# winlaic/ZipVoice

Hardware: AMD Instinct MI355X
Metric: generated mel-frames/s (whole job) + RTF, ZipVoice 123M N_steps=16 batch=32/GPU (higher is better)
Workload: dtype bf16; 1 GPU; C2: ZipVoice 123M, N_steps=16, batch=32/GPU x (3 s prompt + 10 s generated; T=1219 frames), CFG g=1.0 (64 decoder rows per GPU), t_shift=0.5; model=zipvoice (zipvoice_base.json, synthetic seeded weights), global_batch=32, seq_len=1219, parallelism=dp1

## Files before the change

### include/zipvoice_hip.h

```cpp
#ifndef ZIPVOICE_HIP_H
#define ZIPVOICE_HIP_H

#include <stdint.h>

#ifdef __cplusplus
extern "C" {
#endif

typedef struct zv_engine* zv_handle;

enum zv_variant { ZV_ZIPVOICE = 0, ZV_DISTILL = 1, ZV_DIALOG = 2, ZV_DIALOG_STEREO = 3 };
enum zv_precision { ZV_FP32 = 0, ZV_BF16 = 1, ZV_MIXED = 2, ZV_FP8 = 3 };

#define ZV_MAX_STACKS 8

typedef struct {
  int variant;
  int precision;
  int feat_dim;
  int num_stacks;
  int downsampling_factor[ZV_MAX_STACKS];
  int num_layers[ZV_MAX_STACKS];
  int cnn_module_kernel[ZV_MAX_STACKS];
  int fm_decoder_dim, fm_decoder_feedforward_dim, fm_decoder_num_heads;
// ... 94 lines not shown
enum zv_stackedge_kind { ZV_SE_DOWNSAMPLE = 0, ZV_SE_UPSAMPLE = 1, ZV_SE_MASK = 2, ZV_SE_ENTRY = 3, ZV_SE_BIASNORM = 4 };
typedef struct {
  int kind, B, L, C, ds, guard, rows_per_group;
  float log_scale;
  const float* x; const float* w; const float* nb; const float* orig; const float* rowvec;
  const uint8_t* mask;
  float* out;
  uint8_t* mout;
  uint16_t* h; uint16_t* l; uint16_t* h2; uint16_t* l2; int64_t ldact;
  uint8_t* q2; uint8_t* qs2; int64_t ldq;
  int launch[8];
  int num_cus;
} zv_stackedge_check_args;
int zv_stackedge_check(zv_stackedge_check_args* a);

enum zv_bigvgan_check_kind { ZV_BV_FILTER = 0, ZV_BV_ACT = 1, ZV_BV_CONV = 2, ZV_BV_CONVT = 3, ZV_BV_AVG = 4,
                             ZV_BV_POST = 5, ZV_BV_IM2COL = 6, ZV_BV_STEP = 7 };
typedef struct {
  int kind, split, mode, guard;
  int B, Lmax, Ls, halo, scale;
  int C, Cout, ks, d, u, n, layout, flag;
  float div, sub, bias0;
  unsigned stale;
  const int* lens;
  const float* x; const float* x1; const float* x2;
  const float* w; const float* bias; const float* alpha; const float* ibeta;
  const float* w2; const float* bias2; const float* alpha2; const float* ibeta2;
  const float* taps; const float* resid;
  const uint16_t* ah; const uint16_t* al;
  float* out; uint16_t* oh; uint16_t* ol; int64_t ld;
// ... 125 lines not shown
```

### zipvoice_amd/csrc/zv_checks.inc

```
#pragma once

namespace {

struct ChkDev {
  std::vector<void*> ptrs;
  void* raw(size_t bytes) {
    void* p = nullptr;
    ZV_CHECK(ZV_BLOCKING(hipMalloc(&p, bytes + 256)));
    ptrs.push_back(p);
    return p;
  }
  template <typename T> T* make(size_t n) { return reinterpret_cast<T*>(raw(n * sizeof(T))); }
  template <typename T> T* zero(size_t n) {
    T* d = make<T>(n);
    ZV_CHECK(ZV_BLOCKING(hipMemset(d, 0, n * sizeof(T))));
    return d;
  }
  template <typename T> T* up(const T* host, size_t n) {
    T* d = make<T>(n);
    ZV_CHECK(ZV_BLOCKING(hipMemcpy(d, host, n * sizeof(T), hipMemcpyHostToDevice)));
    return d;
  }
  template <typename T> void down(T* host, const T* dev, size_t n) {
    ZV_CHECK(ZV_BLOCKING(hipMemcpy(host, dev, n * sizeof(T), hipMemcpyDeviceToHost)));
// ... 696 lines not shown
    }
    ZV_LAUNCH_CHECK();
    ZV_CHECK(ZV_BLOCKING(hipDeviceSynchronize()));
    dev.down(a->out, o, (size_t)(M + 2 * G) * C);
    down16(a->h, h, M); down16(a->l, l, M); down16(a->h2, h2, M); down16(a->l2, l2, M);
    if (q2) {
      dev.down(a->q2, q2, (size_t)(M + 2 * G) * a->ldq);
      dev.down(a->qs2, qs2, (size_t)(M + 2 * G) * ldqs);
    }
  }
  memcpy(a->launch, rec, sizeof(rec));
  a->num_cus = zv_num_cus();
  ZV_API_END
}

}

namespace {
inline unsigned chk_hash(size_t i, unsigned seed) {
  unsigned x = (unsigned)i * 2654435761u ^ (seed * 0x9E3779B9u + 0x7F4A7C15u);
  x ^= x >> 13; x *= 0x5bd1e995u; x ^= x >> 15;
  return x;
}
inline uint16_t chk_stale16(size_t i, unsigned seed) {
  const unsigned x = chk_hash(i, seed);
  return (uint16_t)(0x3C00u | (x & 0x3FFu) | ((x >> 16 & 1u) << 15));
}
inline float chk_stale32(size_t i, unsigned seed) {
  const unsigned x = chk_hash(i, seed);
  return ((x >> 20 & 1u) ? -1.f : 1.f) * (1.f + (float)(x & 0xFFFFu) / 16384.f);
// ... 258 lines not shown
```

### zipvoice_amd/csrc/zv_elem.inc

```
#pragma once
#include "zv_common.h"
#include "zv_gemm.inc"

__global__ void zv_build_input_kernel(const float* x, const float* tc, const float* sc,
                                      bf16* oh, bf16* ol, long ld, int B, int T, int Fx, int Ft,
                                      int Fs, int ncopies, int zero_speech_uncond) {
  const int Fin = Fx + Ft + Fs;
  const long total = (long)ncopies * B * T * Fin;
  for (long idx = blockIdx.x * (long)blockDim.x + threadIdx.x; idx < total;
       idx += (long)gridDim.x * blockDim.x) {
    const int f = (int)(idx % Fin);
    const long row = idx / Fin;
    const long bt = row % ((long)B * T);
    const int copy = (int)(row / ((long)B * T));
    const bool uncond = (ncopies == 2 && copy == 0);
    float v;
    if (f < Fx) v = x[bt * Fx + f];
    else if (f < Fx + Ft) v = uncond ? 0.f : tc[bt * Ft + (f - Fx)];
    else v = (uncond && zero_speech_uncond) ? 0.f : sc[bt * Fs + (f - Fx - Ft)];
    split_store(oh, ol, row * ld + f, v);
  }
}

__global__ __launch_bounds__(256) void zv_build_input4_kernel(
// ... 659 lines not shown

__global__ void zv_mask_downsample_kernel(const uint8_t* in, uint8_t* out, int B, int L,
                                          int dL, int ds) {
  const int idx = blockIdx.x * blockDim.x + threadIdx.x;
  if (idx >= B * dL) return;
  const int b = idx / dL, i = idx % dL;
  out[idx] = in[(long)b * L + (long)i * ds];
}

__global__ void zv_copy_u8_kernel(const uint8_t* in, uint8_t* out, long n, int copies) {
  const long idx = blockIdx.x * (long)blockDim.x + threadIdx.x;
  if (idx >= n * copies) return;
  out[idx] = in[idx % n];
}

__global__ void zv_embed_kernel(const int64_t* tok, const float* table, bf16* oh, bf16* ol,
                                long ld, long n, int C) {
  const long total = n * C;
  for (long idx = blockIdx.x * (long)blockDim.x + threadIdx.x; idx < total;
       idx += (long)gridDim.x * blockDim.x) {
    const long r = idx / C;
    const int c = (int)(idx % C);
    split_store(oh, ol, r * ld + c, table[tok[r] * C + c]);
  }
}

__global__ void zv_spk_add_kernel(float* emb, const int8_t* spk, const float* table, long n,
                                  int C) {
  const long total = n * C;
  for (long idx = blockIdx.x * (long)blockDim.x + threadIdx.x; idx < total;
// ... 36 lines not shown
```

### zipvoice_amd/csrc/zv_engine.hip

```cpp
#include <math.h>
#include <stdlib.h>
#include <string.h>

#include <map>
#include <memory>
#include <mutex>
#include <string>
#include <exception>
#include <functional>
#include <tuple>
#include <vector>


#include "zv_common.h"
#include "zv_gemm.inc"
#include "zv_gemm256.inc"
#include "zv_ffn.inc"
#include "zv_attn.inc"
#include "zv_elem.inc"
#include "zv_flash.inc"
#include "zv_flash2.inc"
#include "zv_weights.inc"
#include "zv_linear.inc"
#include "../../include/zipvoice_hip.h"
// ... 67 lines not shown
    a.ld = ld;
    a.h = with16 ? h.get<bf16>((size_t)rows * ld) : nullptr;
    a.l = split ? l.get<bf16>((size_t)rows * ld) : nullptr;
    if (fp8) {
      a.ldq = round_up(cols ? cols : ld, MX8_KSTEP);
      a.q = q.get<uint8_t>((size_t)rows * a.ldq);
      a.qs = qs.get<uint8_t>((size_t)rows * a.ldq / MX8_BLOCK);
    }
    return a;
  }
  size_t bytes() const { return h.bytes + l.bytes + q.bytes + qs.bytes; }
};

struct Workspace {
  DBuf main, dsrc, cur, temb0, temb1, tstack, tvec, gvec, posP, mask2, maskds, vout, stats;
  ActBuf xin, main_a, dsrc_a, cur_a, qkp, W, hidden, na_y, na_xt, na_o, sa_vt, sa_o, glu, dw, emb;
  ActBuf cur8;
  ActBuf dwo;
  DBuf ffn_part, ffn_flag;
  static constexpr int POSP_STACKS = 8;
  DBuf posPs[POSP_STACKS];
  struct PosPKey { int L = -1, nl = 0; const void* w = nullptr; const void* buf = nullptr; };
  PosPKey posk[POSP_STACKS];
  size_t bytes() const {
    size_t s = 0;
    for (const DBuf& b : posPs) s += b.bytes;
    for (const DBuf* b : {&main, &dsrc, &cur, &temb0, &temb1, &tstack, &tvec, &gvec, &posP, &mask2,
                          &maskds, &vout, &stats, &ffn_part, &ffn_flag})
      s += b->bytes;
    for (const ActBuf* b : {&xin, &main_a, &dsrc_a, &cur_a, &qkp, &W, &hidden, &na_y, &na_xt, &na_o,
                            &sa_vt, &sa_o, &glu, &dw, &emb, &cur8, &dwo})
      s += b->bytes();
    return s;
  }
};

constexpr int ZV_STREAM_SET = 4;
struct StreamSet { hipStream_t s[ZV_STREAM_SET] = {}; int dev = -1; };
static std::mutex g_stream_pool_mu;
static std::vector<StreamSet>& stream_pool_free() { static std::vector<StreamSet> v; return v; }
static StreamSet acquire_stream_set() {
  int dev = 0;
  ZV_CHECK(hipGetDevice(&dev));
  {
    std::lock_guard<std::mutex> lock(g_stream_pool_mu);
    auto& fr = stream_pool_free();
    for (size_t i = 0; i < fr.size(); ++i)
      if (fr[i].dev == dev) {
// ... 48 lines not shown
    auto envi = [](const char* k, int d) { const char* v = getenv(k); return v ? atoi(v) : d; };
    materialize_attn = envi("ZV_ATTN_MATERIALIZE", 0) == 1;
    graph_mode = envi("ZV_GRAPH", 2);
    sa_tp = envi("ZV_SA_TP", 1);
    fp8_fuse = envi("ZV_FP8_FUSE", 7);
    ffn_fused = envi("ZV_FFN", 2);
    ffn_min_rows = envi("ZV_FFN_MIN_ROWS", 15000);
    ffn_persist = envi("ZV_FFN_PERSIST", 1);
    split_streams = envi("ZV_SPLIT_STREAMS", 3);
    split_min_rows = envi("ZV_SPLIT_MIN_ROWS", 8192);
    mixed_sa = envi("ZV_MIXED_SA", 1) != 0;
    attn_b2 = envi("ZV_ATTN2", 1) != 0 && (cfg.precision == ZV_BF16 || cfg.precision == ZV_FP8);
    attn_b2_dec = attn_b2 || (envi("ZV_ATTN2", 1) != 0 && cfg.precision == ZV_MIXED);
    attn2_exact = envi("ZV_ATTN2_EXACT", 0) != 0;
    glu_dw = envi("ZV_GLU_DW", 1);
  }
  struct GraphKey {
    int B, T, N, has_pad;
    float g, t0, t1, shift;
    int cfg_mode;
    unsigned long gen;
    bool operator<(const GraphKey& o) const {
      return std::tie(B, T, N, has_pad, g, t0, t1, shift, cfg_mode, gen) <
             std::tie(o.B, o.T, o.N, o.has_pad, o.g, o.t0, o.t1, o.shift, o.cfg_mode, o.gen);
    }
  };
  static constexpr size_t MAX_GRAPHS = 8, MAX_SEEN = 256;
  struct GraphEntry { hipGraphExec_t exec; unsigned long last_use; };
  std::map<GraphKey, GraphEntry> graphs;
  std::map<GraphKey, int> graph_seen;
  unsigned long graph_clock = 0;
  hipStream_t gstream = nullptr;
  hipEvent_t gev_in = nullptr, gev_out = nullptr;
  DBuf gx, gtc, gsc, gpad, ggrows;
  int graph_mode = 2;
  bool posp_reuse = false;
  bool io_split = false;

  int ffn_persist = 1;
  long dec_rows_N = 0;
  void attach_ffn_scratch(FfnParams& q, Workspace& ws) {
    if (!ffn_persist) return;
    const int cus = zv_num_cus();
    q.part = ws.ffn_part.get<float>((size_t)cus * FFN_PART_FLOATS);
    unsigned* fl = ws.ffn_flag.get<unsigned>((size_t)cus + 64);
    q.flag = fl;
    q.part_slots = cus;
  }
  void ffn_site(FfnParams q, Workspace& ws, hipStream_t s, const char* tag) {
    attach_ffn_scratch(q, ws);
    launch_ffn(q, s, tag);
// ... 605 lines not shown
                           has_next ? cur_a.l : nullptr, (long)D, temb, L, M,
                           q2 ? c8.q : nullptr, q2 ? c8.qs : nullptr, q2 ? c8.ldq : 0L);
      else
        hipLaunchKernelGGL(zv_biasnorm_bypass_kernel, dim3(cdiv(M, 4)), dim3(256), 0, s, cur, src,
                           W.norm_bias, W.norm_log_scale, W.bypass, src, src_a.h, src_a.l,
                           (float*)nullptr, has_next ? cur_a.h : nullptr,
                           has_next ? cur_a.l : nullptr,
                           (long)D, temb, L, M, D,
                           q2 ? c8.q : nullptr, q2 ? c8.qs : nullptr, q2 ? c8.ldq : 0L);
    }
    ZV_LAUNCH_CHECK();
  }

  template <int SPLIT>
  void stack(const ZipformerW& Z, const StackW& S, int si, Workspace& ws, float* src, Act src_a, int B,
             int L, const uint8_t* pad, const float* temb, hipStream_t s) {
    const long M = (long)B * L;
    const bool split = SPLIT == 3;
    float* cur = ws.cur.get<float>(M * Z.dim);
    Act cur_a = ws.cur_a.get(M, Z.dim, split);
    hipLaunchKernelGGL(zv_stack_entry_kernel, grid1d(M * Z.dim), dim3(256), 0, s, src, temb,
                       (float*)nullptr, src_a.h, src_a.l, cur_a.h, cur_a.l, (long)Z.dim, M,
                       Z.dim, L);
    ZV_LAUNCH_CHECK();
    const int R = 2 * L - 1, HPD = Z.heads * Z.pd, nl = (int)S.layers.size();
    const size_t pn = (size_t)std::max(nl, 1) * R * HPD;
    const bool own = si >= 0 && si < Workspace::POSP_STACKS;
    float* posP = own ? ws.posPs[si].get<float>(pn) : ws.posP.get<float>(pn);
    bool reuse = false;
    if (own) {
      Workspace::PosPKey& k = ws.posk[si];
      reuse = posp_reuse && k.L == L && k.nl == nl && k.w == S.pos_w_all && k.buf == posP;
      k = Workspace::PosPKey{L, nl, S.pos_w_all, posP};
    }
    if (!reuse) {
      hipLaunchKernelGGL(zv_posp_kernel, dim3((unsigned)cdiv((long)nl * R * HPD, 256L)), dim3(256), 0, s, S.pos_w_all, posP,
                         L, nl, HPD, Z.pos_dim);
      ZV_LAUNCH_CHECK();
    }
    for (size_t li = 0; li < S.layers.size(); ++li)
      layer<SPLIT>(Z, S.layers[li], ws, src, src_a, cur, cur_a, B, L, pad,
                   posP + li * (size_t)R * HPD, temb, li + 1 < S.layers.size(), s, li > 0);
  }

  template <int SPLIT>
  void zipformer(const ZipformerW& Z, Workspace& ws, Act xin, int sidx, int N, int T,
                 const uint8_t* pad, const float* t, const float* g, float* out, hipStream_t s) {
    const long M = (long)N * T;
    const int D = Z.dim;
    const bool split = SPLIT == 3;
    float* main = ws.main.get<float>(M * D);
    const bool ios = SPLIT == 1 && io_split;
    Act main_a = ws.main_a.get(M, D, split || ios);
    {
      Out o; o.C = main; o.ldc = D;
      if (ios) linear<3>(Z.in_proj[sidx], xin, M, o, s);
      else linear<SPLIT>(Z.in_proj[sidx], xin, M, o, s);
    }
    float* tstack = nullptr;
    if (Z.has_time) {
      const int E = Z.temb_dim;
      float* e0 = ws.temb0.get<float>((size_t)N * 2 * E);
      float* e1 = ws.temb1.get<float>((size_t)N * 2 * E);
      hipLaunchKernelGGL(zv_timestep_embed_kernel, grid1d(N * E), dim3(256), 0, s, t, temb_freqs,
                         e0, N, E);
      ZV_LAUNCH_CHECK();
      if (Z.has_guid) {
        hipLaunchKernelGGL(zv_timestep_embed_kernel, grid1d(N * E), dim3(256), 0, s, g,
                           temb_freqs, e1, N, E);
        ZV_LAUNCH_CHECK();
        small_linear(Z.guid, e1, E, N, e0, E, 0, e0, s);
      }
      small_linear(Z.te0, e0, E, N, e1, 2 * E, 0, nullptr, s);
      small_linear(Z.te2, e1, 2 * E, N, e0, E, 1, nullptr, s);
      tstack = ws.tstack.get<float>(Z.stacks.size() * (size_t)N * D);
      for (size_t si = 0; si < Z.stacks.size(); ++si)
        small_linear(Z.stacks[si].time_emb, e0, E, N, tstack + si * (size_t)N * D, D, 1, nullptr,
                     s);
    }
    for (size_t si = 0; si < Z.stacks.size(); ++si) {
      const StackW& S = Z.stacks[si];
      const float* te = tstack ? tstack + si * (size_t)N * D : nullptr;
      if (S.ds == 1) {
        stack<SPLIT>(Z, S, (int)si, ws, main, main_a, N, T, pad, te, s);
      } else {
        const int dL = (T + S.ds - 1) / S.ds;
        float* d = ws.dsrc.get<float>((size_t)N * dL * D);
        Act d_a = ws.dsrc_a.get((long)N * dL, D, split || ios);
        hipLaunchKernelGGL(zv_downsample_kernel, grid1d((long)N * dL * D), dim3(256), 0, s, main, d,
                           N, T, dL, D, S.ds, S.ds_w);
        ZV_LAUNCH_CHECK();
        uint8_t* pds = nullptr;
        if (pad) {
          pds = ws.maskds.get<uint8_t>((size_t)N * dL);
          hipLaunchKernelGGL(zv_mask_downsample_kernel, grid1d(N * dL), dim3(256), 0, s, pad, pds,
                             N, T, dL, S.ds);
          ZV_LAUNCH_CHECK();
        }
        stack<SPLIT>(Z, S, (int)si, ws, d, d_a, N, dL, pds, te, s);
        if (D % 4 == 0 && 256 % (D / 4) == 0) {
          const long rows_per_block = 4L * (256 / (D / 4));
          hipLaunchKernelGGL(zv_upsample_combine_kernel,
                             dim3((unsigned)((M + rows_per_block - 1) / rows_per_block)), dim3(256), 0,
                             s, main, d, S.combiner, main, N, T, dL, D, S.ds);
        } else {
          hipLaunchKernelGGL(zv_upsample_combine_any_kernel, grid1d(M * D), dim3(256), 0, s, main, d,
                             S.combiner, main, N, T, dL, D, S.ds);
        }
        ZV_LAUNCH_CHECK();
      }
    }
    ZV_REQUIRE(Z.stacks.back().ds == 1, "last stack must have downsampling factor 1");
    {
      Out o; o.C = out; o.ldc = Z.out_proj[sidx].N;
      if (ios) linear<3>(Z.out_proj[sidx], main_a, M, o, s);
      else linear<SPLIT>(Z.out_proj[sidx], main_a, M, o, s);
    }
  }

  Act build_xin(Workspace& ws, const float* x, const float* tc, const float* sc, int B, int T,
                int Fx, int copies, int zero_speech, hipStream_t s) {
    const int Ft = cfg.feat_dim, Fin = 2 * Fx + Ft;
    const bool split = cfg.precision == ZV_FP32 || cfg.precision == ZV_MIXED;
    const long N = (long)copies * B;
    Act xin = ws.xin.get(N * T, round_up(Fin, 64), split);
    if (Fx % 4 == 0 && Ft % 4 == 0 && xin.ld % 4 == 0)
      hipLaunchKernelGGL(zv_build_input4_kernel, grid1d(N * T * Fin / 4), dim3(256), 0, s, x, tc, sc,
                         xin.h, xin.l, xin.ld, B, T, Fx, Ft, Fx, copies, zero_speech);
    else
      hipLaunchKernelGGL(zv_build_input_kernel, grid1d(N * T * Fin), dim3(256), 0, s, x, tc, sc,
                         xin.h, xin.l, xin.ld, B, T, Fx, Ft, Fx, copies, zero_speech);
    ZV_LAUNCH_CHECK();
    return xin;
  }

  void decoder_rows(Workspace& ws, Act xin, int sidx, int N, int T, const uint8_t* pad,
                    const float* t, const float* g, float* out, hipStream_t s) {
    if (cfg.precision == ZV_FP32) zipformer<3>(dec, ws, xin, sidx, N, T, pad, t, g, out, s);
    else zipformer<1>(dec, ws, xin, sidx, N, T, pad, t, g, out, s);
  }

  void decoder(Act xin, int Fin, int N, int T, const uint8_t* pad, const float* t, const float* g,
               float* out, hipStream_t s) {
    int sidx = 0;
    if (stereo()) sidx = (Fin == dec.in_proj[0].K) ? 0 : 1;
    ZV_REQUIRE(Fin == dec.in_proj[sidx].K, "decoder input width does not match in_proj");
    io_split = cfg.precision == ZV_MIXED;
    if (split_streams < 2 || N < 2 || (long)N * T < split_min_rows) {
      decoder_rows(ws_dec, xin, sidx, N, T, pad, t, g, out, s);
      return;
    }
    const int parts = std::min(split_streams, std::min(N, MAX_SPLIT));
    if (!split_fork) {
      ZV_CHECK(ZV_BLOCKING(hipEventCreateWithFlags(&split_fork, hipEventDisableTiming)));
      for (int i = 0; i < MAX_SPLIT - 1; ++i)
        ZV_CHECK(ZV_BLOCKING(hipEventCreateWithFlags(&split_join[i], hipEventDisableTiming)));
    }
    for (int i = 1; i < parts; ++i)
      if (!split_stream[i - 1]) split_stream[i - 1] = engine_stream(i - 1);
    const int outN = dec.out_proj[sidx].N;
    ZV_CHECK(hipEventRecord(split_fork, s));
    dec_rows_N = N;
    int r0 = 0;
    for (int i = 0; i < parts; ++i) {
      const int n = N / parts + (i < N % parts ? 1 : 0);
      const long rows = (long)r0 * T;
      Act xi = xin;
      xi.h += rows * xin.ld;
      if (xin.l) xi.l += rows * xin.ld;
      const bool serial = g_zv_prof.on;
      hipStream_t si = (i == 0 || serial) ? s : split_stream[i - 1];
      if (i > 0 && !serial) ZV_CHECK(hipStreamWaitEvent(si, split_fork, 0));
      Workspace* wsi = i == 0 ? &ws_dec : &ws_split[i - 1];
      const uint8_t* padi = pad ? pad + rows : nullptr;
      const float* ti = t + r0;
      const float* gi = g ? g + r0 : nullptr;
      float* oi = out + rows * outN;
      try {
        decoder_rows(*wsi, xi, sidx, n, T, padi, ti, gi, oi, si);
      } catch (...) {
        dec_rows_N = 0;
        throw;
      }
      r0 += n;
    }
    dec_rows_N = 0;
    for (int i = 1; i < parts && !g_zv_prof.on; ++i) {
      ZV_CHECK(hipEventRecord(split_join[i - 1], split_stream[i - 1]));
      ZV_CHECK(hipStreamWaitEvent(s, split_join[i - 1], 0));
    }
  }

  void velocity(float t, float gscale, const float* grows, bool cfg_rows, const float* x,
                const float* tc, const float* sc, const uint8_t* pad, int B, int T, float* vout,
                bool euler, float dt, hipStream_t s) {
    const int Fx = stereo() ? 2 * cfg.feat_dim : cfg.feat_dim;
    const int Fin = 2 * Fx + cfg.feat_dim;
    const bool cfg_on = !distill() && (grows ? cfg_rows : gscale != 0.0f);
    const int copies = cfg_on ? 2 : 1;
    const int N = copies * B;
    float g = gscale, gmul = 1.0f;
    int zero_speech = 0;
    if (cfg_on) {
      if (t > 0.5f) zero_speech = 1;
      else { g = gscale * 2.0f; gmul = 2.0f; }
    }
    Act xin = build_xin(ws_dec, x, tc, sc, B, T, Fx, copies, zero_speech, s);
    const uint8_t* padN = pad;
    if (pad && copies == 2) {
      uint8_t* p2 = ws_dec.mask2.get<uint8_t>((size_t)N * T);
      hipLaunchKernelGGL(zv_copy_u8_kernel, grid1d((long)N * T), dim3(256), 0, s, pad, p2,
                         (long)B * T, 2);
      ZV_LAUNCH_CHECK();
      padN = p2;
    }
    float* tv = ws_dec.tvec.get<float>(N);
    hipLaunchKernelGGL(zv_fill_kernel, dim3(cdiv(N, 256)), dim3(256), 0, s, tv, t, N);
    ZV_LAUNCH_CHECK();
    const float* gv = nullptr;
    if (distill()) {
      if (grows) {
        gv = grows;
      } else {
        float* g1 = ws_dec.gvec.get<float>(N);
        hipLaunchKernelGGL(zv_fill_kernel, dim3(cdiv(N, 256)), dim3(256), 0, s, g1, gscale, N);
        ZV_LAUNCH_CHECK();
        gv = g1;
      }
    }
    const long n = (long)B * T * Fx;
    float* v = (copies == 2 || euler) ? ws_dec.vout.get<float>((size_t)N * T * Fx) : vout;
    decoder(xin, Fin, N, T, padN, tv, gv, v, s);
    const float* gr = cfg_on ? grows : nullptr;
    if (euler) {
      hipLaunchKernelGGL(zv_euler_update_kernel, grid1d(n), dim3(256), 0, s, const_cast<float*>(x),
                         v, n, copies == 2 ? 1 : 0, g, dt, gr, gmul, (long)T * Fx);
      ZV_LAUNCH_CHECK();
    } else if (copies == 2) {
      hipLaunchKernelGGL(zv_cfg_combine_kernel, grid1d(n), dim3(256), 0, s, vout, v, n, g, gr,
                         gmul, (long)T * Fx);
      ZV_LAUNCH_CHECK();
    }
  }

  void euler_loop(float* x, const float* tc, const float* sc, const uint8_t* pad, int B, int T,
                  const std::vector<float>& ts, float g, const float* grows, bool cfg_rows,
                  hipStream_t s) {
    const int num_step = (int)ts.size() - 1;
    struct Reset { bool& f; ~Reset() { f = false; } } reset{posp_reuse};
    for (int k = 0; k < num_step; ++k) {
      posp_reuse = k > 0;
      velocity(ts[k], g, grows, cfg_rows, x, tc, sc, pad, B, T, nullptr, true, ts[k + 1] - ts[k],
               s);
    }
  }

  void euler_sample(float* x, const float* tc, const float* sc, const uint8_t* pad, int B, int T,
                    int num_step, float g, const float* grows, bool cfg_rows, float t0, float t1,
                    float shift, hipStream_t s) {
    const std::vector<float> ts = time_steps(t0, t1, num_step, shift);
    bool graph = graph_mode != 0 && !g_zv_prof.on;
    if (graph && graph_mode == 2) {
      const bool cfg_on = !distill() && (grows ? cfg_rows : g != 0.0f);
      const long N = (cfg_on ? 2L : 1L) * B;
      graph = !(split_streams >= 2 && N >= 2 && N * T >= split_min_rows);
    }
// ... 179 lines not shown
  ZV_REQUIRE(max_batch > 0 && max_frames > 0, "bad reservation");
  const int Fx = h->stereo() ? 2 * h->cfg.feat_dim : h->cfg.feat_dim;
  const size_t nx = (size_t)max_batch * max_frames * Fx;
  const size_t nt = (size_t)max_batch * max_frames * h->cfg.feat_dim;
  DBuf bx, btc, bv, bpad;
  const float *x = bx.get<float>(nx), *tc = btc.get<float>(nt);
  float* v = bv.get<float>(nx);
  const uint8_t* pad = bpad.get<uint8_t>((size_t)max_batch * max_frames);
  (void)h->gx.get<float>(nx);
  (void)h->gtc.get<float>(nt);
  (void)h->gsc.get<float>(nx);
  (void)h->gpad.get<uint8_t>((size_t)max_batch * max_frames);
  (void)h->ggrows.get<float>((size_t)max_batch);
  h->velocity(0.25f, 1.0f, nullptr, false, x, tc, x, pad, max_batch, max_frames, v, false,
              0.f, nullptr);
  ZV_CHECK(ZV_BLOCKING(hipDeviceSynchronize()));
  ZV_API_END
}

int zv_attn_fallbacks(zv_handle h, int reset, int64_t* host_counts) {
  ZV_API_BEGIN
  check_ready(h);
  ZV_REQUIRE(host_counts != nullptr, "null counts");
  unsigned c[4] = {0, 0, 0, 0};
  ZV_CHECK(ZV_BLOCKING(hipDeviceSynchronize()));
  ZV_CHECK(ZV_BLOCKING(hipMemcpy(c, h->attn_fallback, sizeof c, hipMemcpyDeviceToHost)));
  for (int i = 0; i < 3; ++i) host_counts[i] = c[i];
  if (reset) ZV_CHECK(ZV_BLOCKING(hipMemset(h->attn_fallback, 0, sizeof c)));
  ZV_API_END
}
// ... 326 lines not shown
```

### zipvoice_amd/engine.py

```python
from __future__ import annotations

import ctypes
import os
from typing import Dict, Optional

import numpy as np
import torch

from .config import ModelConfig
from .weights import check_state_dict

LIB_NAME = "libzipvoice_hip.so"
LIB_PATH = os.path.join(os.path.dirname(os.path.abspath(__file__)), LIB_NAME)
LIB_F16_PATH = os.path.join(os.path.dirname(os.path.abspath(__file__)), "libzipvoice_hip_f16.so")
MAX_STACKS = 8
VARIANT_ID = {"zipvoice": 0, "zipvoice_distill": 1, "zipvoice_dialog": 2,
              "zipvoice_dialog_stereo": 3}
PRECISION_ID = {"fp32": 0, "bf16": 1}
MODES = {"fp32": ("bf16", 0), "bf16": ("bf16", 1), "fp16": ("f16", 2),
         "fp16_plain": ("f16", 1), "bf16_mixed": ("bf16", 2), "fp8": ("bf16", 3)}


class ZvConfig(ctypes.Structure):
    _fields_ = [
# ... 41 lines not shown
    _fields_ = [(n, ctypes.c_int) for n in ("B", "L", "C", "ks", "split", "guard")] + [
        (n, ctypes.c_void_p) for n in ("g", "w", "bias")] + [
        ("ldin", ctypes.c_int64),
        ("Oh", ctypes.c_void_p), ("Ol", ctypes.c_void_p), ("ldout", ctypes.c_int64),
        ("q", ctypes.c_void_p), ("qs", ctypes.c_void_p), ("ldq", ctypes.c_int64),
        ("launch", ctypes.c_int * 8), ("num_cus", ctypes.c_int)]


class ZvStackedgeCheckArgs(ctypes.Structure):
    _fields_ = [(n, ctypes.c_int) for n in ("kind", "B", "L", "C", "ds", "guard", "rows_per_group")] + [
        ("log_scale", ctypes.c_float)] + [
        (n, ctypes.c_void_p) for n in ("x", "w", "nb", "orig", "rowvec", "mask", "out", "mout",
                                       "h", "l", "h2", "l2")] + [
        ("ldact", ctypes.c_int64),
        ("q2", ctypes.c_void_p), ("qs2", ctypes.c_void_p), ("ldq", ctypes.c_int64),
        ("launch", ctypes.c_int * 8), ("num_cus", ctypes.c_int)]


class ZvBigvganCheckArgs(ctypes.Structure):
    _fields_ = [(n, ctypes.c_int) for n in ("kind", "split", "mode", "guard", "B", "Lmax", "Ls", "halo", "scale",
                                            "C", "Cout", "ks", "d", "u", "n", "layout", "flag")] + [
        (n, ctypes.c_float) for n in ("div", "sub", "bias0")] + [
        ("stale", ctypes.c_uint)] + [
        (n, ctypes.c_void_p) for n in ("lens", "x", "x1", "x2", "w", "bias", "alpha", "ibeta", "w2", "bias2",
                                       "alpha2", "ibeta2", "taps", "resid", "ah", "al", "out", "oh", "ol")] + [
        ("ld", ctypes.c_int64),
        ("launch", ctypes.c_int * 8), ("num_cus", ctypes.c_int)]


_P = ctypes.c_void_p
# ... 3 lines not shown
    "zv_last_error": (ctypes.c_char_p, []),
    "zv_version": (ctypes.c_char_p, []),
    "zv_create": (_P, [ctypes.POINTER(ZvConfig)]),
    "zv_destroy": (None, [_P]),
    "zv_set_weight": (_I, [_P, ctypes.c_char_p, _P, ctypes.c_int64]),
    "zv_finalize": (_I, [_P]),
    "zv_reserve": (_I, [_P, _I, _I]),
    "zv_device_bytes": (ctypes.c_int64, [_P]),
    "zv_profile": (_I, [_I]),
    "zv_bench_gemm": (_I, [_I, _I, _I, _I, _I, _I, ctypes.POINTER(ctypes.c_float)]),
    "zv_gemm_selftest": (_I, [_I, _I, _I, _I, _I, ctypes.POINTER(ctypes.c_float), ctypes.POINTER(ctypes.c_float)]),
    "zv_linear_check": (_I, [ctypes.POINTER(ZvLinearCheckArgs)]),
    "zv_ffn_check": (_I, [ctypes.POINTER(ZvFfnCheckArgs)]),
    "zv_dwconv_check": (_I, [ctypes.POINTER(ZvDwconvCheckArgs)]),
    "zv_stackedge_check": (_I, [ctypes.POINTER(ZvStackedgeCheckArgs)]),
    "zv_bigvgan_check": (_I, [ctypes.POINTER(ZvBigvganCheckArgs)]),
    "zv_profile_report": (_I, [ctypes.c_char_p, _I]),
    "zv_host_block_count": (ctypes.c_int64, []),
    "zv_attn_fallbacks": (_I, [_P, _I, _P]),
    "zv_attn2_check": (_I, [_I, _I, _I, _I, _I, _I, _P, _P, _P, _P, _P, _I, _P, _P]),
    "zv_attn_plan": (_I, [_I, _I, _I, _I, _I, _P, _P, _P, _P]),
    "zv_mx8_quantize": (_I, [_P, _I, _I, _P, _P]),
    "zv_mx8_gemm_check": (_I, [_I, _I, _I, _P, _P, _P, _P, _P]),
    "zv_fm_decoder": (_I, [_P, _P, _P, _P, _P, _P, _P, _I, _I, _I, _P, _P]),
    "zv_velocity": (_I, [_P, _F, _F, _P, _P, _P, _P, _I, _I, _P, _P]),
    "zv_euler_sample": (_I, [_P, _P, _P, _P, _P, _I, _I, _I, _F, _F, _F, _F, _P]),
    "zv_velocity_rows": (_I, [_P, _F, _P, _P, _P, _P, _P, _I, _I, _P, _P]),
    "zv_euler_sample_rows": (_I, [_P, _P, _P, _P, _P, _I, _I, _I, _P, _F, _F, _F, _P]),
    "zv_text_encode": (_I, [_P, _P, _P, _P, _I, _I, _P, _P]),
    "zv_text_condition": (_I, [_P, _P, _I, _I, _P, _P, _I, _P, _P]),
# ... 294 lines not shown
```

Measured before the change: 83150 mel-frames/s.

## Fuse stack boundary upsample/downsample/entry kernels and precompute per-solve time and mask tables

Adds a templated kernel that merges the previous stack's upsample-combine, the next stack's downsample and the stack entry split-store into one pass over the main activations, for 512-wide decoders. The Euler loop also precomputes time embeddings for all steps and the duplicated and downsampled padding masks once per solve instead of once per velocity call. The aim is fewer small elementwise launches and less memory traffic at each stack boundary and each step. The cost is extra workspace buffers, a second downsample buffer to avoid aliasing, and more dispatch logic with fallbacks.

```diff
diff --git a/include/zipvoice_hip.h b/include/zipvoice_hip.h
--- a/include/zipvoice_hip.h
+++ b/include/zipvoice_hip.h
@@ -132,6 +132,17 @@
 } zv_stackedge_check_args;
 int zv_stackedge_check(zv_stackedge_check_args* a);
 
+typedef struct {
+  int a, b, B, L, C, guard;
+  const float* x; const float* d; const float* sc; const float* w; const float* rowvec;
+  float* main;
+  float* dout;
+  uint16_t* h; uint16_t* l; uint16_t* h2; uint16_t* l2; int64_t ldact;
+  int launch[8];
+  int num_cus;
+} zv_stackfuse_check_args;
+int zv_stackfuse_check(zv_stackfuse_check_args* a);
+
 enum zv_bigvgan_check_kind { ZV_BV_FILTER = 0, ZV_BV_ACT = 1, ZV_BV_CONV = 2, ZV_BV_CONVT = 3, ZV_BV_AVG = 4,
                              ZV_BV_POST = 5, ZV_BV_IM2COL = 6, ZV_BV_STEP = 7 };
 typedef struct {
diff --git a/zipvoice_amd/csrc/zv_checks.inc b/zipvoice_amd/csrc/zv_checks.inc
--- a/zipvoice_amd/csrc/zv_checks.inc
+++ b/zipvoice_amd/csrc/zv_checks.inc
@@ -734,6 +734,55 @@
   ZV_API_END
 }
 
+int zv_stackfuse_check(zv_stackfuse_check_args* a) {
+  ZV_API_BEGIN
+  ZV_REQUIRE(a && a->a >= 1 && a->b >= 1 && a->B > 0 && a->L > 0 && a->C > 0 && a->C % 4 == 0 && a->guard >= 0 &&
+                 a->x && a->h && a->h2 && a->ldact >= a->C && a->ldact % 4 == 0,
+             "zv_stackfuse_check: bad arguments");
+  ZV_REQUIRE(a->a == 1 || (a->d && a->sc && a->main), "zv_stackfuse_check: a > 1 needs d, sc and main");
+  ZV_REQUIRE(a->b == 1 || (a->w && a->dout), "zv_stackfuse_check: b > 1 needs w and dout");
+  const int B = a->B, L = a->L, C = a->C, G = a->guard;
+  const int dLa = (L + a->a - 1) / a->a, dLb = (L + a->b - 1) / a->b;
+  const long M = (long)B * L, Me = (long)B * dLb;
+  ChkDev dev;
+  hipStream_t s = nullptr;
+  float* main = nullptr;
+  float* mbuf = nullptr;
+  if (a->a > 1) {
+    std::vector<float> hc(a->main, a->main + (size_t)(M + 2 * G) * C);
+    memcpy(&hc[(size_t)G * C], a->x, (size_t)M * C * sizeof(float));
+    mbuf = dev.up(hc.data(), hc.size());
+    main = mbuf + (size_t)G * C;
+  } else {
+    main = dev.up(a->x, (size_t)M * C);
+  }
+  const float* d = a->a > 1 ? dev.up(a->d, (size_t)B * dLa * C) : nullptr;
+  const float* sc = a->a > 1 ? dev.up(a->sc, (size_t)C) : nullptr;
+  const float* w = a->b > 1 ? dev.up(a->w, (size_t)a->b) : nullptr;
+  const float* rv = a->rowvec ? dev.up(a->rowvec, (size_t)B * C) : nullptr;
+  float* dout = a->b > 1 ? dev.up(a->dout, (size_t)(Me + 2 * G) * C) : nullptr;
+  auto up16 = [&](uint16_t* p) {
+    return p ? reinterpret_cast<bf16*>(dev.up(p, (size_t)(Me + 2 * G) * a->ldact)) : nullptr;
+  };
+  auto in16 = [&](bf16* p) { return p ? p + (size_t)G * a->ldact : nullptr; };
+  bf16 *h = up16(a->h), *l = up16(a->l), *h2 = up16(a->h2), *l2 = up16(a->l2);
+  int blocks = 0;
+  const bool ran = launch_stack_fuse(a->a, a->b, C, main, d, sc, dout ? dout + (size_t)G * C : nullptr, w, rv,
+                                     in16(h), in16(l), in16(h2), in16(l2), (long)a->ldact, B, L, s, &blocks);
+  ZV_REQUIRE(ran, "zv_stackfuse_check: no fused kernel for this factor pair and width");
+  ZV_CHECK(ZV_BLOCKING(hipDeviceSynchronize()));
+  const int rec[8] = {a->a, a->b, blocks, 256, 0, 0, 0, 0};
+  if (mbuf) dev.down(a->main, mbuf, (size_t)(M + 2 * G) * C);
+  if (dout) dev.down(a->dout, dout, (size_t)(Me + 2 * G) * C);
+  auto down16 = [&](uint16_t* p, bf16* q) {
+    if (p) dev.down(p, reinterpret_cast<uint16_t*>(q), (size_t)(Me + 2 * G) * a->ldact);
+  };
+  down16(a->h, h); down16(a->l, l); down16(a->h2, h2); down16(a->l2, l2);
+  memcpy(a->launch, rec, sizeof(rec));
+  a->num_cus = zv_num_cus();
+  ZV_API_END
+}
+
 }
 
 namespace {
diff --git a/zipvoice_amd/csrc/zv_elem.inc b/zipvoice_amd/csrc/zv_elem.inc
--- a/zipvoice_amd/csrc/zv_elem.inc
+++ b/zipvoice_amd/csrc/zv_elem.inc
@@ -697,6 +697,88 @@
   out[idx] = in[idx % n];
 }
 
+template <int A, int B>
+__global__ __launch_bounds__(256) void zv_stack_fuse_kernel(
+    float* main, const float* dprev, const float* sc, float* dnext, const float* w,
+    const float* rowvec, bf16* srch, bf16* srcl, bf16* curh, bf16* curl, long ldact, int N, int L) {
+  constexpr int C = 512, G = A > B ? A : B;
+  const int c = (threadIdx.x & 127) * 4;
+  const int ngl = (L + G - 1) / G;
+  const long grp = blockIdx.x * 2L + (threadIdx.x >> 7);
+  if (grp >= (long)N * ngl) return;
+  const int n = (int)(grp / ngl), l0 = (int)(grp - (long)n * ngl) * G;
+  const int dLa = (L + A - 1) / A, dLb = (L + B - 1) / B;
+  float wk[B];
+#pragma unroll
+  for (int k = 0; k < B; ++k) wk[k] = B > 1 ? w[k] : 1.0f;
+  f32x4 rv = {0.f, 0.f, 0.f, 0.f};
+  if (rowvec) rv = *reinterpret_cast<const f32x4*>(rowvec + (long)n * C + c);
+  f32x4 m[G];
+#pragma unroll
+  for (int j = 0; j < G; ++j) {
+    const int l = l0 + j < L ? l0 + j : L - 1;
+    m[j] = *reinterpret_cast<const f32x4*>(main + ((long)n * L + l) * C + c);
+  }
+  if constexpr (A > 1) {
+    const f32x4 scv = *reinterpret_cast<const f32x4*>(sc + c);
+    f32x4 u[G];
+#pragma unroll
+    for (int j = 0; j < G; ++j) {
+      const int l = l0 + j < L ? l0 + j : L - 1;
+      u[j] = *reinterpret_cast<const f32x4*>(dprev + ((long)n * dLa + l / A) * C + c);
+    }
+#pragma unroll
+    for (int j = 0; j < G; ++j) m[j] = m[j] + (u[j] - m[j]) * scv;
+#pragma unroll
+    for (int j = 0; j < G; ++j)
+      if (l0 + j < L) *reinterpret_cast<f32x4*>(main + ((long)n * L + l0 + j) * C + c) = m[j];
+  }
+  auto entry = [&](long row, const f32x4& v) {
+    f32x4 y = v;
+    if (rowvec) y = y + rv;
+    float vv[4] = {v[0], v[1], v[2], v[3]}, yv[4] = {y[0], y[1], y[2], y[3]};
+    store_split4(srch, srcl, row * ldact + c, vv);
+    store_split4(curh, curl, row * ldact + c, yv);
+  };
+  if constexpr (B > 1) {
+#pragma unroll
+    for (int q = 0; q < G / B; ++q)
+      if (l0 + q * B < L) {
+        f32x4 acc = {0.f, 0.f, 0.f, 0.f};
+#pragma unroll
+        for (int k = 0; k < B; ++k) acc += m[q * B + k] * wk[k];
+        const long row = (long)n * dLb + l0 / B + q;
+        *reinterpret_cast<f32x4*>(dnext + row * C + c) = acc;
+        entry(row, acc);
+      }
+  } else {
+#pragma unroll
+    for (int j = 0; j < G; ++j)
+      if (l0 + j < L) entry((long)n * L + l0 + j, m[j]);
+  }
+}
+
+static bool launch_stack_fuse(int a, int b, int C, float* main, const float* dprev, const float* sc,
+                              float* dnext, const float* w, const float* rowvec, bf16* srch, bf16* srcl,
+                              bf16* curh, bf16* curl, long ldact, int N, int L, hipStream_t s,
+                              int* grid_blocks = nullptr) {
+  if (C != 512 || N <= 0 || L <= 0 || ldact % 4 != 0) return false;
+  const int G = a > b ? a : b;
+  const long groups = (long)N * ((L + G - 1) / G);
+  const dim3 grid((unsigned)((groups + 1) / 2));
+#define ZV_STACK_FUSE_CASE(A_, B_)                                                                   \
+  if (a == A_ && b == B_)                                                                            \
+    hipLaunchKernelGGL((zv_stack_fuse_kernel<A_, B_>), grid, dim3(256), 0, s, main, dprev, sc, dnext, \
+                       w, rowvec, srch, srcl, curh, curl, ldact, N, L);                              \
+  else
+  ZV_STACK_FUSE_CASE(1, 2) ZV_STACK_FUSE_CASE(2, 4) ZV_STACK_FUSE_CASE(4, 2) ZV_STACK_FUSE_CASE(2, 1)
+    return false;
+#undef ZV_STACK_FUSE_CASE
+  ZV_LAUNCH_CHECK();
+  if (grid_blocks) *grid_blocks = (int)grid.x;
+  return true;
+}
+
 __global__ void zv_embed_kernel(const int64_t* tok, const float* table, bf16* oh, bf16* ol,
                                 long ld, long n, int C) {
   const long total = n * C;
diff --git a/zipvoice_amd/csrc/zv_engine.hip b/zipvoice_amd/csrc/zv_engine.hip
--- a/zipvoice_amd/csrc/zv_engine.hip
+++ b/zipvoice_amd/csrc/zv_engine.hip
@@ -105,6 +105,8 @@
 
 struct Workspace {
   DBuf main, dsrc, cur, temb0, temb1, tstack, tvec, gvec, posP, mask2, maskds, vout, stats;
+  DBuf dsrc2;
+  DBuf solve_t, solve_temb, solve_mask;
   ActBuf xin, main_a, dsrc_a, cur_a, qkp, W, hidden, na_y, na_xt, na_o, sa_vt, sa_o, glu, dw, emb;
   ActBuf cur8;
   ActBuf dwo;
@@ -117,12 +119,29 @@
     size_t s = 0;
     for (const DBuf& b : posPs) s += b.bytes;
     for (const DBuf* b : {&main, &dsrc, &cur, &temb0, &temb1, &tstack, &tvec, &gvec, &posP, &mask2,
-                          &maskds, &vout, &stats, &ffn_part, &ffn_flag})
+                          &maskds, &vout, &stats, &ffn_part, &ffn_flag, &dsrc2, &solve_t, &solve_temb,
+                          &solve_mask})
       s += b->bytes;
     for (const ActBuf* b : {&xin, &main_a, &dsrc_a, &cur_a, &qkp, &W, &hidden, &na_y, &na_xt, &na_o,
                             &sa_vt, &sa_o, &glu, &dw, &emb, &cur8, &dwo})
       s += b->bytes();
     return s;
+  }
+};
+
+struct SolveTables {
+  const float* temb = nullptr;
+  size_t stack_stride = 0;
+  int D = 0;
+  const uint8_t* pad2 = nullptr;
+  const uint8_t* padds[ZV_MAX_STACKS] = {};
+  int dL[ZV_MAX_STACKS] = {};
+  SolveTables rows_from(int r0) const {
+    SolveTables o = *this;
+    if (temb) o.temb += (size_t)r0 * D;
+    for (int si = 0; si < ZV_MAX_STACKS; ++si)
+      if (padds[si]) o.padds[si] += (size_t)r0 * dL[si];
+    return o;
   }
 };
 
@@ -201,6 +220,8 @@
     attn_b2_dec = attn_b2 || (envi("ZV_ATTN2", 1) != 0 && cfg.precision == ZV_MIXED);
     attn2_exact = envi("ZV_ATTN2_EXACT", 0) != 0;
     glu_dw = envi("ZV_GLU_DW", 1);
+    stack_fuse = envi("ZV_STACK_FUSE", 1) != 0;
+    solve_tables = envi("ZV_SOLVE_TABLES", 1) != 0;
   }
   struct GraphKey {
     int B, T, N, has_pad;
@@ -222,6 +243,9 @@
   DBuf gx, gtc, gsc, gpad, ggrows;
   int graph_mode = 2;
   bool posp_reuse = false;
+  bool stack_fuse = true;
+  bool solve_tables = true;
+  SolveTables tab;
   bool io_split = false;
 
   int ffn_persist = 1;
@@ -857,15 +881,17 @@
 
   template <int SPLIT>
   void stack(const ZipformerW& Z, const StackW& S, int si, Workspace& ws, float* src, Act src_a, int B,
-             int L, const uint8_t* pad, const float* temb, hipStream_t s) {
+             int L, const uint8_t* pad, const float* temb, hipStream_t s, bool entry_done = false) {
     const long M = (long)B * L;
     const bool split = SPLIT == 3;
     float* cur = ws.cur.get<float>(M * Z.dim);
     Act cur_a = ws.cur_a.get(M, Z.dim, split);
-    hipLaunchKernelGGL(zv_stack_entry_kernel, grid1d(M * Z.dim), dim3(256), 0, s, src, temb,
-                       (float*)nullptr, src_a.h, src_a.l, cur_a.h, cur_a.l, (long)Z.dim, M,
-                       Z.dim, L);
-    ZV_LAUNCH_CHECK();
+    if (!entry_done) {
+      hipLaunchKernelGGL(zv_stack_entry_kernel, grid1d(M * Z.dim), dim3(256), 0, s, src, temb,
+                         (float*)nullptr, src_a.h, src_a.l, cur_a.h, cur_a.l, (long)Z.dim, M,
+                         Z.dim, L);
+      ZV_LAUNCH_CHECK();
+    }
     const int R = 2 * L - 1, HPD = Z.heads * Z.pd, nl = (int)S.layers.size();
     const size_t pn = (size_t)std::max(nl, 1) * R * HPD;
     const bool own = si >= 0 && si < Workspace::POSP_STACKS;
@@ -886,9 +912,45 @@
                    posP + li * (size_t)R * HPD, temb, li + 1 < S.layers.size(), s, li > 0);
   }
 
+  void time_embed(const ZipformerW& Z, Workspace& ws, int rows, const float* t, const float* g,
+                  float* out, size_t stride, hipStream_t s) {
+    const int E = Z.temb_dim, D = Z.dim;
+    float* e0 = ws.temb0.get<float>((size_t)rows * 2 * E);
+    float* e1 = ws.temb1.get<float>((size_t)rows * 2 * E);
+    hipLaunchKernelGGL(zv_timestep_embed_kernel, grid1d(rows * E), dim3(256), 0, s, t, temb_freqs,
+                       e0, rows, E);
+    ZV_LAUNCH_CHECK();
+    if (Z.has_guid) {
+      hipLaunchKernelGGL(zv_timestep_embed_kernel, grid1d(rows * E), dim3(256), 0, s, g,
+                         temb_freqs, e1, rows, E);
+      ZV_LAUNCH_CHECK();
+      small_linear(Z.guid, e1, E, rows, e0, E, 0, e0, s);
+    }
+    small_linear(Z.te0, e0, E, rows, e1, 2 * E, 0, nullptr, s);
+    small_linear(Z.te2, e1, 2 * E, rows, e0, E, 1, nullptr, s);
+    for (size_t si = 0; si < Z.stacks.size(); ++si)
+      small_linear(Z.stacks[si].time_emb, e0, E, rows, out + si * stride, D, 1, nullptr, s);
+  }
+
+  void upsample_combine(const StackW& S, float* main, const float* d, int N, int T, int D, hipStream_t s) {
+    const long M = (long)N * T;
+    const int dL = (T + S.ds - 1) / S.ds;
+    if (D % 4 == 0 && 256 % (D / 4) == 0) {
+      const long rows_per_block = 4L * (256 / (D / 4));
+      hipLaunchKernelGGL(zv_upsample_combine_kernel,
+                         dim3((unsigned)((M + rows_per_block - 1) / rows_per_block)), dim3(256), 0,
+                         s, main, d, S.combiner, main, N, T, dL, D, S.ds);
+    } else {
+      hipLaunchKernelGGL(zv_upsample_combine_any_kernel, grid1d(M * D), dim3(256), 0, s, main, d,
+                         S.combiner, main, N, T, dL, D, S.ds);
+    }
+    ZV_LAUNCH_CHECK();
+  }
+
   template <int SPLIT>
   void zipformer(const ZipformerW& Z, Workspace& ws, Act xin, int sidx, int N, int T,
-                 const uint8_t* pad, const float* t, const float* g, float* out, hipStream_t s) {
+                 const uint8_t* pad, const float* t, const float* g, float* out, hipStream_t s,
+                 const SolveTables& tb = SolveTables{}) {
     const long M = (long)N * T;
     const int D = Z.dim;
     const bool split = SPLIT == 3;
@@ -900,57 +962,57 @@
       if (ios) linear<3>(Z.in_proj[sidx], xin, M, o, s);
       else linear<SPLIT>(Z.in_proj[sidx], xin, M, o, s);
     }
-    float* tstack = nullptr;
-    if (Z.has_time) {
-      const int E = Z.temb_dim;
-      float* e0 = ws.temb0.get<float>((size_t)N * 2 * E);
-      float* e1 = ws.temb1.get<float>((size_t)N * 2 * E);
-      hipLaunchKernelGGL(zv_timestep_embed_kernel, grid1d(N * E), dim3(256), 0, s, t, temb_freqs,
-                         e0, N, E);
-      ZV_LAUNCH_CHECK();
-      if (Z.has_guid) {
-        hipLaunchKernelGGL(zv_timestep_embed_kernel, grid1d(N * E), dim3(256), 0, s, g,
-                           temb_freqs, e1, N, E);
-        ZV_LAUNCH_CHECK();
-        small_linear(Z.guid, e1, E, N, e0, E, 0, e0, s);
-      }
-      small_linear(Z.te0, e0, E, N, e1, 2 * E, 0, nullptr, s);
-      small_linear(Z.te2, e1, 2 * E, N, e0, E, 1, nullptr, s);
-      tstack = ws.tstack.get<float>(Z.stacks.size() * (size_t)N * D);
-      for (size_t si = 0; si < Z.stacks.size(); ++si)
-        small_linear(Z.stacks[si].time_emb, e0, E, N, tstack + si * (size_t)N * D, D, 1, nullptr,
-                     s);
-    }
+    const float* tstack = nullptr;
+    size_t tstride = (size_t)N * D;
+    if (Z.has_time && tb.temb) {
+      tstack = tb.temb;
+      tstride = tb.stack_stride;
+    } else if (Z.has_time) {
+      float* ts = ws.tstack.get<float>(Z.stacks.size() * (size_t)N * D);
+      time_embed(Z, ws, N, t, g, ts, tstride, s);
+      tstack = ts;
+    }
+    float* dprev = nullptr;
     for (size_t si = 0; si < Z.stacks.size(); ++si) {
       const StackW& S = Z.stacks[si];
-      const float* te = tstack ? tstack + si * (size_t)N * D : nullptr;
-      if (S.ds == 1) {
-        stack<SPLIT>(Z, S, (int)si, ws, main, main_a, N, T, pad, te, s);
+      const float* te = tstack ? tstack + si * tstride : nullptr;
+      const int a = si > 0 ? Z.stacks[si - 1].ds : 1, b = S.ds;
+      const int dL = (T + b - 1) / b;
+      float* d = nullptr;
+      Act d_a;
+      if (b != 1) {
+        d = stack_fuse && dprev && dprev == ws.dsrc.p ? ws.dsrc2.get<float>((size_t)N * dL * D) : ws.dsrc.get<float>((size_t)N * dL * D);
+        d_a = ws.dsrc_a.get((long)N * dL, D, split || ios);
+      }
+      bool fused = false;
+      if (stack_fuse && si > 0) {
+        Act cur_a = ws.cur_a.get((long)N * dL, D, split);
+        const Act& src_a = b != 1 ? d_a : main_a;
+        fused = launch_stack_fuse(a, b, D, main, dprev, Z.stacks[si - 1].combiner, d, S.ds_w, te, src_a.h,
+                                  src_a.l, cur_a.h, cur_a.l, (long)D, N, T, s);
+      }
+      if (!fused && dprev) upsample_combine(Z.stacks[si - 1], main, dprev, N, T, D, s);
+      if (b == 1) {
+        stack<SPLIT>(Z, S, (int)si, ws, main, main_a, N, T, pad, te, s, fused);
+        dprev = nullptr;
       } else {
-        const int dL = (T + S.ds - 1) / S.ds;
-        float* d = ws.dsrc.get<float>((size_t)N * dL * D);
-        Act d_a = ws.dsrc_a.get((long)N * dL, D, split || ios);
-        hipLaunchKernelGGL(zv_downsample_kernel, grid1d((long)N * dL * D), dim3(256), 0, s, main, d,
-                           N, T, dL, D, S.ds, S.ds_w);
-        ZV_LAUNCH_CHECK();
-        uint8_t* pds = nullptr;
-        if (pad) {
-          pds = ws.maskds.get<uint8_t>((size_t)N * dL);
-          hipLaunchKernelGGL(zv_mask_downsample_kernel, grid1d(N * dL), dim3(256), 0, s, pad, pds,
-                             N, T, dL, S.ds);
+        if (!fused) {
+          hipLaunchKernelGGL(zv_downsample_kernel, grid1d((long)N * dL * D), dim3(256), 0, s, main, d,
+                             N, T, dL, D, b, S.ds_w);
           ZV_LAUNCH_CHECK();
         }
-        stack<SPLIT>(Z, S, (int)si, ws, d, d_a, N, dL, pds, te, s);
-        if (D % 4 == 0 && 256 % (D / 4) == 0) {
-          const long rows_per_block = 4L * (256 / (D / 4));
-          hipLaunchKernelGGL(zv_upsample_combine_kernel,
-                             dim3((unsigned)((M + rows_per_block - 1) / rows_per_block)), dim3(256), 0,
-                             s, main, d, S.combiner, main, N, T, dL, D, S.ds);
-        } else {
-          hipLaunchKernelGGL(zv_upsample_combine_any_kernel, grid1d(M * D), dim3(256), 0, s, main, d,
-                             S.combiner, main, N, T, dL, D, S.ds);
+        const uint8_t* pds = nullptr;
+        if (pad && si < ZV_MAX_STACKS && tb.padds[si]) {
+          pds = tb.padds[si];
+        } else if (pad) {
+          uint8_t* p = ws.maskds.get<uint8_t>((size_t)N * dL);
+          hipLaunchKernelGGL(zv_mask_downsample_kernel, grid1d(N * dL), dim3(256), 0, s, pad, p,
+                             N, T, dL, b);
+          ZV_LAUNCH_CHECK();
+          pds = p;
         }
-        ZV_LAUNCH_CHECK();
+        stack<SPLIT>(Z, S, (int)si, ws, d, d_a, N, dL, pds, te, s, fused);
+        dprev = d;
       }
     }
     ZV_REQUIRE(Z.stacks.back().ds == 1, "last stack must have downsampling factor 1");
@@ -978,9 +1040,9 @@
   }
 
   void decoder_rows(Workspace& ws, Act xin, int sidx, int N, int T, const uint8_t* pad,
-                    const float* t, const float* g, float* out, hipStream_t s) {
-    if (cfg.precision == ZV_FP32) zipformer<3>(dec, ws, xin, sidx, N, T, pad, t, g, out, s);
-    else zipformer<1>(dec, ws, xin, sidx, N, T, pad, t, g, out, s);
+                    const float* t, const float* g, float* out, hipStream_t s, const SolveTables& tb) {
+    if (cfg.precision == ZV_FP32) zipformer<3>(dec, ws, xin, sidx, N, T, pad, t, g, out, s, tb);
+    else zipformer<1>(dec, ws, xin, sidx, N, T, pad, t, g, out, s, tb);
   }
 
   void decoder(Act xin, int Fin, int N, int T, const uint8_t* pad, const float* t, const float* g,
@@ -990,7 +1052,7 @@
     ZV_REQUIRE(Fin == dec.in_proj[sidx].K, "decoder input width does not match in_proj");
     io_split = cfg.precision == ZV_MIXED;
     if (split_streams < 2 || N < 2 || (long)N * T < split_min_rows) {
-      decoder_rows(ws_dec, xin, sidx, N, T, pad, t, g, out, s);
+      decoder_rows(ws_dec, xin, sidx, N, T, pad, t, g, out, s, tab);
       return;
     }
     const int parts = std::min(split_streams, std::min(N, MAX_SPLIT));
@@ -1016,11 +1078,11 @@
       if (i > 0 && !serial) ZV_CHECK(hipStreamWaitEvent(si, split_fork, 0));
       Workspace* wsi = i == 0 ? &ws_dec : &ws_split[i - 1];
       const uint8_t* padi = pad ? pad + rows : nullptr;
-      const float* ti = t + r0;
+      const float* ti = t ? t + r0 : nullptr;
       const float* gi = g ? g + r0 : nullptr;
       float* oi = out + rows * outN;
       try {
-        decoder_rows(*wsi, xi, sidx, n, T, padi, ti, gi, oi, si);
+        decoder_rows(*wsi, xi, sidx, n, T, padi, ti, gi, oi, si, tab.rows_from(r0));
       } catch (...) {
         dec_rows_N = 0;
         throw;
@@ -1050,18 +1112,24 @@
     }
     Act xin = build_xin(ws_dec, x, tc, sc, B, T, Fx, copies, zero_speech, s);
     const uint8_t* padN = pad;
-    if (pad && copies == 2) {
+    if (pad && copies == 2 && tab.pad2) {
+      padN = tab.pad2;
+    } else if (pad && copies == 2) {
       uint8_t* p2 = ws_dec.mask2.get<uint8_t>((size_t)N * T);
       hipLaunchKernelGGL(zv_copy_u8_kernel, grid1d((long)N * T), dim3(256), 0, s, pad, p2,
                          (long)B * T, 2);
       ZV_LAUNCH_CHECK();
       padN = p2;
     }
-    float* tv = ws_dec.tvec.get<float>(N);
-    hipLaunchKernelGGL(zv_fill_kernel, dim3(cdiv(N, 256)), dim3(256), 0, s, tv, t, N);
-    ZV_LAUNCH_CHECK();
+    const bool have_temb = tab.temb != nullptr;
+    float* tv = nullptr;
+    if (!have_temb) {
+      tv = ws_dec.tvec.get<float>(N);
+      hipLaunchKernelGGL(zv_fill_kernel, dim3(cdiv(N, 256)), dim3(256), 0, s, tv, t, N);
+      ZV_LAUNCH_CHECK();
+    }
     const float* gv = nullptr;
-    if (distill()) {
+    if (distill() && !have_temb) {
       if (grows) {
         gv = grows;
       } else {
@@ -1086,13 +1154,93 @@
     }
   }
 
+  static constexpr int RESERVE_STEPS = 32;
+  void reserve_solve_tables(int B, int T) {
+    if (!solve_tables) return;
+    const size_t N = 2 * (size_t)B, rows = RESERVE_STEPS * N;
+    if (dec.has_time) {
+      (void)ws_dec.solve_t.get<float>(rows * 2);
+      (void)ws_dec.solve_temb.get<float>(dec.stacks.size() * rows * dec.dim);
+      (void)ws_dec.temb0.get<float>(rows * 2 * dec.temb_dim);
+      (void)ws_dec.temb1.get<float>(rows * 2 * dec.temb_dim);
+    }
+    size_t total = round_up((long)(N * T), 256);
+    for (const StackW& S : dec.stacks)
+      if (S.ds != 1) total += round_up((long)(N * ((T + S.ds - 1) / S.ds)), 256);
+    (void)ws_dec.solve_mask.get<uint8_t>(total);
+  }
+
   void euler_loop(float* x, const float* tc, const float* sc, const uint8_t* pad, int B, int T,
                   const std::vector<float>& ts, float g, const float* grows, bool cfg_rows,
                   hipStream_t s) {
     const int num_step = (int)ts.size() - 1;
-    struct Reset { bool& f; ~Reset() { f = false; } } reset{posp_reuse};
+    struct Reset {
+      bool& f; SolveTables& t;
+      ~Reset() { f = false; t = SolveTables{}; }
+    } reset{posp_reuse, tab};
+    tab = SolveTables{};
+    const float* temb_all = nullptr;
+    size_t temb_step = 0;
+    if (solve_tables && num_step > 0) {
+      const bool cfg_on = !distill() && (grows ? cfg_rows : g != 0.0f);
+      const int copies = cfg_on ? 2 : 1, N = copies * B, D = dec.dim;
+      if (dec.has_time) {
+        const int rows = num_step * N;
+        float* tall = ws_dec.solve_t.get<float>((size_t)rows * 2);
+        float* gall = dec.has_guid ? tall + rows : nullptr;
+        float* table = ws_dec.solve_temb.get<float>(dec.stacks.size() * (size_t)rows * D);
+        for (int k = 0; k < num_step; ++k) {
+          hipLaunchKernelGGL(zv_fill_kernel, dim3(cdiv(N, 256)), dim3(256), 0, s, tall + (size_t)k * N, ts[k], N);
+          ZV_LAUNCH_CHECK();
+          if (gall && grows)
+            ZV_CHECK(hipMemcpyAsync(gall + (size_t)k * N, grows, (size_t)N * sizeof(float),
+                                    hipMemcpyDeviceToDevice, s));
+        }
+        if (gall && !grows) {
+          hipLaunchKernelGGL(zv_fill_kernel, dim3(cdiv(rows, 256)), dim3(256), 0, s, gall, g, rows);
+          ZV_LAUNCH_CHECK();
+        }
+        time_embed(dec, ws_dec, rows, tall, gall, table, (size_t)rows * D, s);
+        temb_all = table;
+        temb_step = (size_t)N * D;
+        tab.stack_stride = (size_t)rows * D;
+        tab.D = D;
+      }
+      if (pad) {
+        const size_t nst = std::min(dec.stacks.size(), (size_t)ZV_MAX_STACKS);
+        size_t off[ZV_MAX_STACKS] = {}, total = copies == 2 ? round_up((long)N * T, 256) : 0;
+        bool first[ZV_MAX_STACKS] = {};
+        for (size_t si = 0; si < nst; ++si) {
+          const int ds = dec.stacks[si].ds;
+          if (ds == 1) continue;
+          tab.dL[si] = (T + ds - 1) / ds;
+          size_t sj = 0;
+          while (sj < si && dec.stacks[sj].ds != ds) ++sj;
+          first[si] = sj == si;
+          off[si] = first[si] ? total : off[sj];
+          if (first[si]) total += round_up((long)N * tab.dL[si], 256);
+        }
+        uint8_t* mb = ws_dec.solve_mask.get<uint8_t>(total);
+        const uint8_t* padN = pad;
+        if (copies == 2) {
+          hipLaunchKernelGGL(zv_copy_u8_kernel, grid1d((long)N * T), dim3(256), 0, s, pad, mb, (long)B * T, 2);
+          ZV_LAUNCH_CHECK();
+          tab.pad2 = padN = mb;
+        }
+        for (size_t si = 0; si < nst; ++si) {
+          if (dec.stacks[si].ds == 1) continue;
+          if (first[si]) {
+            hipLaunchKernelGGL(zv_mask_downsample_kernel, grid1d((long)N * tab.dL[si]), dim3(256), 0, s, padN,
+                               mb + off[si], N, T, tab.dL[si], dec.stacks[si].ds);
+            ZV_LAUNCH_CHECK();
+          }
+          tab.padds[si] = mb + off[si];
+        }
+      }
+    }
     for (int k = 0; k < num_step; ++k) {
       posp_reuse = k > 0;
+      if (temb_all) tab.temb = temb_all + (size_t)k * temb_step;
       velocity(ts[k], g, grows, cfg_rows, x, tc, sc, pad, B, T, nullptr, true, ts[k + 1] - ts[k],
                s);
     }
@@ -1302,6 +1450,7 @@
   (void)h->ggrows.get<float>((size_t)max_batch);
   h->velocity(0.25f, 1.0f, nullptr, false, x, tc, x, pad, max_batch, max_frames, v, false,
               0.f, nullptr);
+  h->reserve_solve_tables(max_batch, max_frames);
   ZV_CHECK(ZV_BLOCKING(hipDeviceSynchronize()));
   ZV_API_END
 }
diff --git a/zipvoice_amd/engine.py b/zipvoice_amd/engine.py
--- a/zipvoice_amd/engine.py
+++ b/zipvoice_amd/engine.py
@@ -79,6 +79,13 @@
                                        "h", "l", "h2", "l2")] + [
         ("ldact", ctypes.c_int64),
         ("q2", ctypes.c_void_p), ("qs2", ctypes.c_void_p), ("ldq", ctypes.c_int64),
+        ("launch", ctypes.c_int * 8), ("num_cus", ctypes.c_int)]
+
+
+class ZvStackfuseCheckArgs(ctypes.Structure):
+    _fields_ = [(n, ctypes.c_int) for n in ("a", "b", "B", "L", "C", "guard")] + [
+        (n, ctypes.c_void_p) for n in ("x", "d", "sc", "w", "rowvec", "main", "dout", "h", "l", "h2", "l2")] + [
+        ("ldact", ctypes.c_int64),
         ("launch", ctypes.c_int * 8), ("num_cus", ctypes.c_int)]
 
 
@@ -112,6 +119,7 @@
     "zv_ffn_check": (_I, [ctypes.POINTER(ZvFfnCheckArgs)]),
     "zv_dwconv_check": (_I, [ctypes.POINTER(ZvDwconvCheckArgs)]),
     "zv_stackedge_check": (_I, [ctypes.POINTER(ZvStackedgeCheckArgs)]),
+    "zv_stackfuse_check": (_I, [ctypes.POINTER(ZvStackfuseCheckArgs)]),
     "zv_bigvgan_check": (_I, [ctypes.POINTER(ZvBigvganCheckArgs)]),
     "zv_profile_report": (_I, [ctypes.c_char_p, _I]),
     "zv_host_block_count": (ctypes.c_int64, []),
```

Result: no change. 83970 mel-frames/s (median of 6 runs) (+1.0%).
